# burchim/AVEC

Hardware: AMD Instinct MI355X
Metric: AV utterances/sec fwd+bwd (audio T=400, video 100x88x88) (higher is better)
Workload: dtype bf16

## Files before the change

### avec_amd/csrc/frontend.hip

```cpp
#include "vec.h"
#include "avec_hip.h"

__global__ __launch_bounds__(256) void mel_frames_kernel(const float* __restrict__ audio, const float* __restrict__ window, float* __restrict__ frames,
                                                         int B, long long L, int F, int n_fft, int win, int hop) {
  const long long total = (long long)B * F * win;
  const int off = (n_fft - win) / 2 - n_fft / 2;
  for (long long i = (long long)blockIdx.x * 256 + threadIdx.x; i < total; i += (long long)gridDim.x * 256) {
    const int n = (int)(i % win); const long long r = i / win; const int f = (int)(r % F); const long long b = r / F;
    long long s = (long long)f * hop + n + off;
    if (s < 0) s = -s; else if (s >= L) s = 2 * (L - 1) - s;
    frames[i] = audio[b * L + s] * window[n];
  }
}
__global__ __launch_bounds__(128) void mel_power_log_kernel(const float* __restrict__ spec, const float* __restrict__ fb, float* __restrict__ out,
                                                            int F, int nb, int n_mels) {
  extern __shared__ float pw[];
  const long long m = blockIdx.x; const int f = (int)(m % F); const long long b = m / F;
  for (int k = threadIdx.x; k < nb; k += 128) { const float re = spec[m * 2 * nb + k], im = spec[m * 2 * nb + nb + k]; pw[k] = re * re + im * im; }
  __syncthreads();
  for (int j = threadIdx.x; j < n_mels; j += 128) {
    float s = 0.f;
    for (int k = 0; k < nb; ++k) s += pw[k] * fb[k * n_mels + j];
    out[(b * n_mels + j) * F + f] = logf(s + 1e-9f);
  }
// ... 12 lines not shown

__global__ __launch_bounds__(256) void specaug_kernel(float* __restrict__ mel, const long long* __restrict__ lens, int B, int n_mels, int F, int mF, int Fp, int mT, float pS,
                                                      const unsigned long long* rng, unsigned stream) {
  const unsigned long long seed = rng[0] + 0x9e3779b97f4a7c15ull * rng[1];
  const long long total = (long long)B * n_mels * F;
  for (long long i = (long long)blockIdx.x * 256 + threadIdx.x; i < total; i += (long long)gridDim.x * 256) {
    const int f = (int)(i % F); const long long r = i / F; const int m = (int)(r % n_mels); const int b = (int)(r / n_mels);
    bool masked = false;
    for (int q = 0; q < mF && !masked; ++q) {
      const float val = rng_uniform(seed, stream, 2 * q) * Fp; const float mn = rng_uniform(seed, stream, 2 * q + 1) * (n_mels - val);
      const int s0 = (int)mn, s1 = (int)mn + (int)val; masked = (m >= s0 && m < s1);
    }
    const int len = lens ? (int)lens[b] : F; const int Tp = (int)(pS * len);
    if (f < len) for (int q = 0; q < mT && !masked; ++q) {
      const unsigned long long id = 1000ull + (unsigned long long)b * 64 + 2 * q;
      const float val = rng_uniform(seed, stream, id) * Tp; const float mn = rng_uniform(seed, stream, id + 1) * (len - val);
      const int s0 = (int)mn, s1 = (int)mn + (int)val; masked = (f >= s0 && f < s1);
    }
    if (masked) mel[i] = 0.f;
  }
}
extern "C" int avec_specaugment(float* mel, const long long* lens, int B, int n_mels, int F, int mF, int Fparam, int mT, float pS,
                                const unsigned long long* rng, unsigned rng_stream, hipStream_t st) {
  AVEC_CHECK_ARG(mel && rng && B > 0 && n_mels > 0 && F > 0, "specaugment: bad arguments");
  long long total = (long long)B * n_mels * F; long long nb = (total + 255) / 256; if (nb > 4096) nb = 4096;
  hipLaunchKernelGGL(specaug_kernel, dim3((unsigned)nb), dim3(256), 0, st, mel, lens, B, n_mels, F, mF, Fparam, mT, pS, rng, rng_stream);
  AVEC_LAUNCH_CHECK(); return 0;
}

__global__ void debug_rng_uniform_kernel(const unsigned long long* rng, unsigned stream, const long long* ids, int n, float* out) {
  const unsigned long long seed = rng[0] + 0x9e3779b97f4a7c15ull * rng[1];
  const int i = blockIdx.x * 256 + threadIdx.x;
  if (i < n) out[i] = rng_uniform(seed, stream, (unsigned long long)ids[i]);
}
extern "C" int avec_debug_rng_uniform(const unsigned long long* rng, unsigned rng_stream, const long long* ids, int n, float* out, hipStream_t st) {
  AVEC_CHECK_ARG(rng && ids && out && n > 0, "debug_rng_uniform: bad arguments");
  hipLaunchKernelGGL(debug_rng_uniform_kernel, dim3((n + 255) / 256), dim3(256), 0, st, rng, rng_stream, ids, n, out);
  AVEC_LAUNCH_CHECK(); return 0;
}

struct StemA { int B, NM, F, C, Fo, To; };

__device__ __forceinline__ void block_channel_add2(float* dst, int C, int c, bool live, float a, float b) {
  __shared__ float red[2][16]; __shared__ int cbase;
  if (threadIdx.x == 0) cbase = c;
  if (threadIdx.x < 32) red[threadIdx.x >> 4][threadIdx.x & 15] = 0.f;
  __syncthreads();
  const int k = c - cbase;
  if (live && k >= 0 && k < 16) { atomicAdd(&red[0][k], a); atomicAdd(&red[1][k], b); }
  else if (live) { atomicAdd(dst + c, a); atomicAdd(dst + C + c, b); }
  __syncthreads();
  if (threadIdx.x < 16 && cbase + (int)threadIdx.x < C && (red[0][threadIdx.x] != 0.f || red[1][threadIdx.x] != 0.f)) {
    atomicAdd(dst + cbase + threadIdx.x, red[0][threadIdx.x]); atomicAdd(dst + C + cbase + threadIdx.x, red[1][threadIdx.x]);
  }
}

template <typename T>
__global__ __launch_bounds__(256) void audio_stem_conv_kernel(const float* __restrict__ mel, const float* __restrict__ w, const float* __restrict__ bias,
                                                              T* __restrict__ y, float* stats, StemA s) {
  int j = blockIdx.x * 256 + threadIdx.x; const int J = s.C * s.Fo;
  const bool live = j < J; if (!live) j = J - 1;
  const int c = j / s.Fo, fo = j % s.Fo;
  float wk[9]; for (int q = 0; q < 9; ++q) wk[q] = w[c * 9 + q];
  const float bb = bias ? bias[c] : 0.f;
  float sum = 0.f, sq = 0.f;
  const long long M = (long long)s.B * s.To;
  for (long long row = blockIdx.y; row < M; row += gridDim.y) {
    const int to = (int)(row % s.To); const long long b = row / s.To;
    float acc = bb;
    for (int kh = 0; kh < 3; ++kh) { const int fi = 2 * fo + kh - 1; if (fi < 0 || fi >= s.NM) continue;
      for (int kw = 0; kw < 3; ++kw) { const int ti = 2 * to + kw - 1; if (ti < 0 || ti >= s.F) continue;
        acc += wk[kh * 3 + kw] * mel[(b * s.NM + fi) * s.F + ti]; } }
    if (live) { stf(y + row * J + j, acc); sum += acc; sq += acc * acc; }
  }
  if (stats) block_channel_add2(stats, s.C, c, live, sum, sq);
}
template <typename T>
__global__ __launch_bounds__(256) void audio_stem_act_kernel(const T* __restrict__ y, const float* __restrict__ ss, T* __restrict__ a, long long M, int J, int Fo, int C) {
  const long long total = M * J;
  for (long long i = (long long)blockIdx.x * 256 + threadIdx.x; i < total; i += (long long)gridDim.x * 256) {
    const int c = (int)((unsigned)(i % (long long)J)) / Fo; stf(a + i, swishf_(ldf(y + i) * ss[c] + ss[C + c]));
  }
}
template <typename T>
__global__ __launch_bounds__(256) void audio_stem_act8_kernel(const T* __restrict__ y, const float* __restrict__ ss, T* __restrict__ a, unsigned n8, unsigned J8, int Fo, int C) {
  for (unsigned i = blockIdx.x * 256 + threadIdx.x; i < n8; i += gridDim.x * 256) {
    const int c = (int)((i % J8) * 8) / Fo; const float sc = ss[c], sh = ss[C + c];
    Raw8<T> r; r.load(y + (long long)i * 8); float v[8]; r.get(v);
#pragma unroll
    for (int e = 0; e < 8; ++e) v[e] = swishf_(v[e] * sc + sh);
    st8<T>(a + (long long)i * 8, v);
  }
}
template <typename T>
__global__ __launch_bounds__(256) void audio_stem_bwd_reduce_kernel(const T* __restrict__ da, const T* __restrict__ y, const float* __restrict__ ss, float* dstats, StemA s) {
  int j = blockIdx.x * 256 + threadIdx.x; const int J = s.C * s.Fo;
  const bool live = j < J; if (!live) j = J - 1;
  const int c = j / s.Fo; const float sc = ss[c], sh = ss[s.C + c], mu = ss[2 * s.C + c], rs = ss[3 * s.C + c];
  float s1 = 0.f, s2 = 0.f; const long long M = (long long)s.B * s.To;
  if (live) for (long long row = blockIdx.y; row < M; row += gridDim.y) {
    const float yy = ldf(y + row * J + j); const float dr = ldf(da + row * J + j) * dswishf_(yy * sc + sh);
    s1 += dr; s2 += dr * (yy - mu) * rs;
  }
  block_channel_add2(dstats, s.C, c, live, s1, s2);
}
template <typename T>
__global__ __launch_bounds__(256) void audio_stem_bwd_params_kernel(const T* __restrict__ da, const T* __restrict__ y, const float* __restrict__ mel, const float* __restrict__ ss,
                                                                    const float* __restrict__ gamma, const float* __restrict__ dstats, const float* count_ptr, float count,
                                                                    float* dw, float* dbias, float* dgamma, float* dbeta, StemA s) {
  int j = blockIdx.x * 256 + threadIdx.x; const int J = s.C * s.Fo;
  const bool live = j < J; if (!live) j = J - 1;
  const int c = j / s.Fo, fo = j % s.Fo; const float inv_n = 1.f / (count_ptr ? *count_ptr : count);
  const float sc = ss[c], sh = ss[s.C + c], mu = ss[2 * s.C + c], rs = ss[3 * s.C + c], g = gamma[c];
  const float m1 = dstats[c] * inv_n, m2 = dstats[s.C + c] * inv_n;
  if (live && blockIdx.y == 0 && fo == 0 && dgamma) { atomicAdd(dgamma + c, dstats[s.C + c]); atomicAdd(dbeta + c, dstats[c]); }
  float aw[9]; for (int q = 0; q < 9; ++q) aw[q] = 0.f; float ab = 0.f;
  const long long M = (long long)s.B * s.To;
  if (live) for (long long row = blockIdx.y; row < M; row += gridDim.y) {
    const int to = (int)(row % s.To); const long long b = row / s.To;
    const float yy = ldf(y + row * J + j); const float dr = ldf(da + row * J + j) * dswishf_(yy * sc + sh);
    const float dy = g * rs * (dr - m1 - (yy - mu) * rs * m2);
    ab += dy;
    for (int kh = 0; kh < 3; ++kh) { const int fi = 2 * fo + kh - 1; if (fi < 0 || fi >= s.NM) continue;
      for (int kw = 0; kw < 3; ++kw) { const int ti = 2 * to + kw - 1; if (ti < 0 || ti >= s.F) continue;
        aw[kh * 3 + kw] += dy * mel[(b * s.NM + fi) * s.F + ti]; } }
  }
  __shared__ float wred[16][10]; __shared__ int wbase;
  if (threadIdx.x == 0) wbase = c;
  if (threadIdx.x < 160) wred[threadIdx.x / 10][threadIdx.x % 10] = 0.f;
  __syncthreads();
  const int kq = c - wbase;
  if (live && kq >= 0 && kq < 16) { for (int q = 0; q < 9; ++q) atomicAdd(&wred[kq][q], aw[q]); atomicAdd(&wred[kq][9], ab); }
  else if (live) { for (int q = 0; q < 9; ++q) atomicAdd(dw + c * 9 + q, aw[q]); if (dbias) atomicAdd(dbias + c, ab); }
  __syncthreads();
  if (threadIdx.x < 160) {
    const int cc = wbase + threadIdx.x / 10, q = threadIdx.x % 10; const float v = wred[threadIdx.x / 10][q];
    if (cc < s.C && v != 0.f) { if (q < 9) atomicAdd(dw + cc * 9 + q, v); else if (dbias) atomicAdd(dbias + cc, v); }
  }
}
#ifndef AVEC_AS_ROWS
#define AVEC_AS_ROWS 16
#endif
static constexpr int AS_ROWS = AVEC_AS_ROWS;
__device__ __forceinline__ void stage_mel_patch(float* patch, const float* mel, long long b, int to, const StemA& s) {
  for (int idx = threadIdx.x; idx < (s.NM + 2) * 3; idx += 256) {
    const int fi = idx / 3 - 1, kw = idx - (fi + 1) * 3; const int ti = 2 * to + kw - 1;
    patch[idx] = (fi >= 0 && fi < s.NM && ti >= 0 && ti < s.F) ? mel[(b * s.NM + fi) * s.F + ti] : 0.f;
  }
}
__device__ __forceinline__ void as_commit(const float* lsum, int n, float* const* dst, int ndst, int W, const ColWs& ws) {
  if (ws.partial) { float* mine = ws_slot(ws, 0, blockIdx.x, gridDim.x, n); for (int i = threadIdx.x; i < n; i += 256) mine[i] = lsum[i]; }
  else for (int i = threadIdx.x; i < n; i += 256) { const int q = i / W; if (dst[q] && lsum[i] != 0.f) atomicAdd(dst[q] + (i - q * W), lsum[i]); }
}
template <typename T>
__global__ __launch_bounds__(256) void audio_stem_conv8_kernel(const float* __restrict__ mel, const float* __restrict__ w, const float* __restrict__ bias,
                                                               T* __restrict__ y, float* stats, StemA s, ColWs ws) {
  extern __shared__ float asm_[];
  float* patch = asm_; float* lw = patch + (s.NM + 2) * 3; float* lsum = lw + s.C * 10;
  const int J = s.C * s.Fo, F8 = s.Fo >> 3, chunks = s.C * F8; const long long M = (long long)s.B * s.To;
  for (int i = threadIdx.x; i < s.C * 10; i += 256) { const int c = i / 10, q = i - c * 10; lw[i] = q < 9 ? w[c * 9 + q] : (bias ? bias[c] : 0.f); }
  for (int i = threadIdx.x; i < 2 * s.C; i += 256) lsum[i] = 0.f;
  for (int rr = 0; rr < AS_ROWS; ++rr) {
    const long long row = (long long)blockIdx.x * AS_ROWS + rr; if (row >= M) break;
    const int to = (int)(row % s.To); const long long b = row / s.To;
    __syncthreads();
    stage_mel_patch(patch, mel, b, to, s);
    __syncthreads();
    for (int ch = threadIdx.x; ch < chunks; ch += 256) {
      const int c = ch / F8, fo0 = (ch - c * F8) * 8; const float* wk = lw + c * 10;
      float acc[8], s1 = 0.f, s2 = 0.f;
#pragma unroll
      for (int e = 0; e < 8; ++e) {
        const float* pp = patch + (2 * (fo0 + e)) * 3; float a = wk[9];
// ... 41 lines not shown
  for (int rr = 0; rr < AS_ROWS; ++rr) {
    const long long row = (long long)blockIdx.x * AS_ROWS + rr; if (row >= M) break;
    const int to = (int)(row % s.To); const long long b = row / s.To;
    __syncthreads();
    stage_mel_patch(patch, mel, b, to, s);
    __syncthreads();
    for (int ch = threadIdx.x; ch < chunks; ch += 256) {
      const int c = ch / F8, fo0 = (ch - c * F8) * 8;
      const float sc = ss[c], sh = ss[s.C + c], mu = ss[2 * s.C + c], rs = ss[3 * s.C + c], g = gamma[c];
      const float m1 = dstats[c] * inv_n, m2 = dstats[s.C + c] * inv_n;
      float d[8], v[8], aw[9], ab = 0.f; ld8<T>(da + row * J + c * s.Fo + fo0, d); ld8<T>(y + row * J + c * s.Fo + fo0, v);
#pragma unroll
      for (int q = 0; q < 9; ++q) aw[q] = 0.f;
#pragma unroll
      for (int e = 0; e < 8; ++e) {
        const float dr = d[e] * dswishf_(v[e] * sc + sh); const float dy = g * rs * (dr - m1 - (v[e] - mu) * rs * m2);
        ab += dy; const float* pp = patch + (2 * (fo0 + e)) * 3;
#pragma unroll
        for (int q = 0; q < 9; ++q) aw[q] += dy * pp[q];
      }
#pragma unroll
      for (int q = 0; q < 9; ++q) atomicAdd(lsum + q * s.C + c, aw[q]);
      atomicAdd(lsum + 9 * s.C + c, ab);
    }
  }
  __syncthreads();
  if (ws.partial) { float* mine = ws_slot(ws, 0, blockIdx.x, gridDim.x, 10 * s.C); for (int i = threadIdx.x; i < 10 * s.C; i += 256) mine[i] = lsum[i]; }
  else for (int i = threadIdx.x; i < 10 * s.C; i += 256) { const int q = i / s.C, c = i - q * s.C; if (q < 9) atomicAdd(dw + c * 9 + q, lsum[i]); else if (dbias) atomicAdd(dbias + c, lsum[i]); }
}
constexpr int AS_NIT = 4;
__device__ __forceinline__ void as_patch51(const float* patch, int fo0, float p[52]) {
  const float4* q = (const float4*)(patch + 6 * fo0);
#pragma unroll
  for (int k = 0; k < 13; ++k) { const float4 t = q[k]; p[4 * k] = t.x; p[4 * k + 1] = t.y; p[4 * k + 2] = t.z; p[4 * k + 3] = t.w; }
}
template <typename T>
__global__ __launch_bounds__(256) void audio_stem_conv8x_kernel(const float* __restrict__ mel, const float* __restrict__ w, const float* __restrict__ bias,
                                                                T* __restrict__ y, float* stats, StemA s, ColWs ws) {
  extern __shared__ __attribute__((aligned(16))) float asm_[];
  float* patch = asm_; float* lsum = patch + (((s.NM + 2) * 3 + 4 + 3) & ~3);
  const int J = s.C * s.Fo, F8 = s.Fo >> 3, chunks = s.C * F8; const long long M = (long long)s.B * s.To;
  int cc[AS_NIT], fo[AS_NIT]; float wk[AS_NIT][10], s1[AS_NIT], s2[AS_NIT];
#pragma unroll
  for (int it = 0; it < AS_NIT; ++it) {
    const int ch = threadIdx.x + 256 * it; const bool ok = ch < chunks; cc[it] = ok ? ch / F8 : -1; fo[it] = ok ? (ch - cc[it] * F8) * 8 : 0; s1[it] = s2[it] = 0.f;
#pragma unroll
    for (int q = 0; q < 10; ++q) wk[it][q] = ok ? (q < 9 ? w[cc[it] * 9 + q] : (bias ? bias[cc[it]] : 0.f)) : 0.f;
  }
  for (int i = threadIdx.x; i < 2 * s.C; i += 256) lsum[i] = 0.f;
  for (int rr = 0; rr < AS_ROWS; ++rr) {
    const long long row = (long long)blockIdx.x * AS_ROWS + rr; if (row >= M) break;
    const int to = (int)(row % s.To); const long long b = row / s.To;
    __syncthreads();
    stage_mel_patch(patch, mel, b, to, s);
    __syncthreads();
#pragma unroll
    for (int it = 0; it < AS_NIT; ++it) {
      if (cc[it] < 0) continue;
      float p[52], acc[8]; as_patch51(patch, fo[it], p);
#pragma unroll
      for (int e = 0; e < 8; ++e) {
        float a = wk[it][9];
#pragma unroll
        for (int q = 0; q < 9; ++q) a += wk[it][q] * p[6 * e + q];
        acc[e] = a; s1[it] += a; s2[it] += a * a;
      }
      st8<T>(y + row * J + cc[it] * s.Fo + fo[it], acc);
    }
  }
  if (!stats) return;
#pragma unroll
  for (int it = 0; it < AS_NIT; ++it) if (cc[it] >= 0) { atomicAdd(lsum + cc[it], s1[it]); atomicAdd(lsum + s.C + cc[it], s2[it]); }
  __syncthreads();
  float* const dst[2] = {stats, stats + s.C}; as_commit(lsum, 2 * s.C, dst, 2, s.C, ws);
}
template <typename T>
__global__ __launch_bounds__(256) void audio_stem_bwd_reduce8x_kernel(const T* __restrict__ da, const T* __restrict__ y, const float* __restrict__ ss, float* dstats, StemA s, ColWs ws) {
  extern __shared__ __attribute__((aligned(16))) float asm_[];
  float* lsum = asm_;
  const int J = s.C * s.Fo, F8 = s.Fo >> 3, chunks = s.C * F8; const long long M = (long long)s.B * s.To;
  int cc[AS_NIT], off[AS_NIT]; float sc[AS_NIT], sh[AS_NIT], mu[AS_NIT], rs[AS_NIT], s1[AS_NIT], s2[AS_NIT];
#pragma unroll
  for (int it = 0; it < AS_NIT; ++it) {
    const int ch = threadIdx.x + 256 * it; const bool ok = ch < chunks; const int c = ok ? ch / F8 : 0; cc[it] = ok ? c : -1; off[it] = c * s.Fo + (ch - c * F8) * 8;
    sc[it] = ss[c]; sh[it] = ss[s.C + c]; mu[it] = ss[2 * s.C + c]; rs[it] = ss[3 * s.C + c]; s1[it] = s2[it] = 0.f;
  }
  for (int i = threadIdx.x; i < 2 * s.C; i += 256) lsum[i] = 0.f;
  for (int rr = 0; rr < AS_ROWS; ++rr) {
    const long long row = (long long)blockIdx.x * AS_ROWS + rr; if (row >= M) break;
    Raw8<T> rd[AS_NIT], rv[AS_NIT];
#pragma unroll
    for (int it = 0; it < AS_NIT; ++it) if (cc[it] >= 0) { rd[it].load(da + row * J + off[it]); rv[it].load(y + row * J + off[it]); }
#pragma unroll
    for (int it = 0; it < AS_NIT; ++it) {
      if (cc[it] < 0) continue;
      float d[8], v[8]; rd[it].get(d); rv[it].get(v);
#pragma unroll
      for (int e = 0; e < 8; ++e) { const float dr = d[e] * dswishf_(v[e] * sc[it] + sh[it]); s1[it] += dr; s2[it] += dr * (v[e] - mu[it]) * rs[it]; }
    }
  }
  __syncthreads();
#pragma unroll
  for (int it = 0; it < AS_NIT; ++it) if (cc[it] >= 0) { atomicAdd(lsum + cc[it], s1[it]); atomicAdd(lsum + s.C + cc[it], s2[it]); }
  __syncthreads();
  float* const dst[2] = {dstats, dstats + s.C}; as_commit(lsum, 2 * s.C, dst, 2, s.C, ws);
}
template <typename T>
__global__ __launch_bounds__(256) void audio_stem_bwd_params8x_kernel(const T* __restrict__ da, const T* __restrict__ y, const float* __restrict__ mel, const float* __restrict__ ss,
                                                                      const float* __restrict__ gamma, const float* __restrict__ dstats, const float* count_ptr, float count,
                                                                      float* dw, float* dbias, float* dgamma, float* dbeta, StemA s, ColWs ws) {
  extern __shared__ __attribute__((aligned(16))) float asm_[];
  float* patch = asm_; float* lsum = patch + (((s.NM + 2) * 3 + 4 + 3) & ~3);
  const int J = s.C * s.Fo, F8 = s.Fo >> 3, chunks = s.C * F8; const long long M = (long long)s.B * s.To;
  const float inv_n = 1.f / (count_ptr ? *count_ptr : count);
  if (blockIdx.x == 0 && dgamma) for (int c = threadIdx.x; c < s.C; c += 256) { atomicAdd(dgamma + c, dstats[s.C + c]); atomicAdd(dbeta + c, dstats[c]); }
  int cc[AS_NIT], fo[AS_NIT]; float sc[AS_NIT], sh[AS_NIT], mu[AS_NIT], A[AS_NIT], m1[AS_NIT], rm2[AS_NIT], aw[AS_NIT][10];
#pragma unroll
  for (int it = 0; it < AS_NIT; ++it) {
    const int ch = threadIdx.x + 256 * it; const bool ok = ch < chunks; const int c = ok ? ch / F8 : 0; cc[it] = ok ? c : -1; fo[it] = ok ? (ch - c * F8) * 8 : 0;
    const float rs = ss[3 * s.C + c];
    sc[it] = ss[c]; sh[it] = ss[s.C + c]; mu[it] = ss[2 * s.C + c]; A[it] = gamma[c] * rs; m1[it] = dstats[c] * inv_n; rm2[it] = rs * dstats[s.C + c] * inv_n;
#pragma unroll
    for (int q = 0; q < 10; ++q) aw[it][q] = 0.f;
  }
  for (int i = threadIdx.x; i < 10 * s.C; i += 256) lsum[i] = 0.f;
  for (int rr = 0; rr < AS_ROWS; ++rr) {
    const long long row = (long long)blockIdx.x * AS_ROWS + rr; if (row >= M) break;
    const int to = (int)(row % s.To); const long long b = row / s.To;
    Raw8<T> rd[AS_NIT], rv[AS_NIT];
#pragma unroll
    for (int it = 0; it < AS_NIT; ++it) if (cc[it] >= 0) { const long long o = row * J + cc[it] * s.Fo + fo[it]; rd[it].load(da + o); rv[it].load(y + o); }
    __syncthreads();
    stage_mel_patch(patch, mel, b, to, s);
    __syncthreads();
#pragma unroll
    for (int it = 0; it < AS_NIT; ++it) {
      if (cc[it] < 0) continue;
      float d[8], v[8], p[52]; rd[it].get(d); rv[it].get(v); as_patch51(patch, fo[it], p);
#pragma unroll
      for (int e = 0; e < 8; ++e) {
        const float dr = d[e] * dswishf_(v[e] * sc[it] + sh[it]); const float dy = A[it] * (dr - m1[it] - (v[e] - mu[it]) * rm2[it]);
        aw[it][9] += dy;
#pragma unroll
        for (int q = 0; q < 9; ++q) aw[it][q] += dy * p[6 * e + q];
      }
    }
  }
  __syncthreads();
#pragma unroll
  for (int it = 0; it < AS_NIT; ++it) if (cc[it] >= 0) {
#pragma unroll
    for (int q = 0; q < 10; ++q) atomicAdd(lsum + q * s.C + cc[it], aw[it][q]);
  }
  __syncthreads();
  if (ws.partial) { float* mine = ws_slot(ws, 0, blockIdx.x, gridDim.x, 10 * s.C); for (int i = threadIdx.x; i < 10 * s.C; i += 256) mine[i] = lsum[i]; }
  else for (int i = threadIdx.x; i < 10 * s.C; i += 256) { const int q = i / s.C, c = i - q * s.C; if (q < 9) atomicAdd(dw + c * 9 + q, lsum[i]); else if (dbias) atomicAdd(dbias + c, lsum[i]); }
}
static bool as8x_ok(const StemA& s) { return s.C * (s.Fo >> 3) <= AS_NIT * 256; }
static bool as8_ok(const StemA& s) { return s.Fo % 8 == 0 && ((size_t)(s.NM + 2) * 3 + (size_t)s.C * 12) * 4 <= 60 * 1024; }
static unsigned as8_blocks(const StemA& s) { return (unsigned)(((long long)s.B * s.To + AS_ROWS - 1) / AS_ROWS); }
static StemA stemA(int B, int NM, int F, int C) { StemA s; s.B = B; s.NM = NM; s.F = F; s.C = C; s.Fo = (NM - 1) / 2 + 1; s.To = (F - 1) / 2 + 1; return s; }
static dim3 stem_grid(const StemA& s) { long long M = (long long)s.B * s.To; unsigned gx = (s.C * s.Fo + 255) / 256; long long gy = 2048 / gx; if (gy > M) gy = M; if (gy < 1) gy = 1; return dim3(gx, (unsigned)gy); }

extern "C" int avec_audio_stem_conv_fwd(int dtype, const float* mel, const float* w, const float* bias, void* y, float* stats, int B, int n_mels, int F, int C, hipStream_t st) {
  AVEC_CHECK_ARG(mel && w && y && B > 0 && n_mels > 0 && F > 0 && C > 0, "audio_stem_conv_fwd: bad arguments");
  StemA s = stemA(B, n_mels, F, C);
  if (as8_ok(s)) {
    const unsigned nb = as8_blocks(s); const ColPlan plan = ColPlan::flat<2>(nb, C, st, stats != nullptr);
    const size_t lds = ((size_t)(n_mels + 2) * 3 + (size_t)C * 12) * 4;
    if (as8x_ok(s)) { const size_t l2 = ((size_t)(((n_mels + 2) * 3 + 4 + 3) & ~3) + (size_t)C * 2) * 4;
      DISPATCH_T(dtype, hipLaunchKernelGGL(audio_stem_conv8x_kernel<T>, dim3(nb), dim3(256), l2, st, mel, w, bias, (T*)y, stats, s, plan.ws)); }
    else
    DISPATCH_T(dtype, hipLaunchKernelGGL(audio_stem_conv8_kernel<T>, dim3(nb), dim3(256), lds, st, mel, w, bias, (T*)y, stats, s, plan.ws));
    AVEC_LAUNCH_CHECK();
    return plan.finish({stats, stats + C}, C, st);
  }
  DISPATCH_T(dtype, hipLaunchKernelGGL(audio_stem_conv_kernel<T>, stem_grid(s), dim3(256), 0, st, mel, w, bias, (T*)y, stats, s));
  AVEC_LAUNCH_CHECK(); return 0;
}
extern "C" int avec_audio_stem_act_fwd(int dtype, const void* y, const float* ss, void* a, int B, int n_mels, int F, int C, hipStream_t st) {
  AVEC_CHECK_ARG(y && ss && a, "audio_stem_act_fwd: null pointer");
  StemA s = stemA(B, n_mels, F, C); long long M = (long long)B * s.To; long long nb = (M * C * s.Fo + 255) / 256; if (nb > 4096) nb = 4096;
  if (s.Fo % 8 == 0 && M * C * s.Fo / 8 < (1ll << 31)) {
    const long long n8 = M * C * s.Fo / 8; long long nb8 = (n8 + 255) / 256; if (nb8 > 8192) nb8 = 8192;
    DISPATCH_T(dtype, hipLaunchKernelGGL(audio_stem_act8_kernel<T>, dim3((unsigned)nb8), dim3(256), 0, st, (const T*)y, ss, (T*)a, (unsigned)n8, (unsigned)(C * s.Fo / 8), s.Fo, C));
    AVEC_LAUNCH_CHECK(); return 0;
  }
  DISPATCH_T(dtype, hipLaunchKernelGGL(audio_stem_act_kernel<T>, dim3((unsigned)nb), dim3(256), 0, st, (const T*)y, ss, (T*)a, M, C * s.Fo, s.Fo, C));
  AVEC_LAUNCH_CHECK(); return 0;
}
extern "C" int avec_audio_stem_bwd(int dtype, const void* da, const void* y, const float* mel, const float* ss, const float* gamma, float* dstats,
                                   const float* count_ptr, float count, int phase, float* dw, float* dbias, float* dgamma, float* dbeta,
                                   int B, int n_mels, int F, int C, hipStream_t st) {
  AVEC_CHECK_ARG(da && y && mel && ss && gamma && dstats && (phase == 0 || (dw != nullptr)), "audio_stem_bwd: bad arguments");
  StemA s = stemA(B, n_mels, F, C);
  if (as8_ok(s)) {
    const unsigned nb = as8_blocks(s);
    if (phase == 0) {
      const ColPlan plan = ColPlan::flat<2>(nb, C, st);
      if (as8x_ok(s)) DISPATCH_T(dtype, hipLaunchKernelGGL(audio_stem_bwd_reduce8x_kernel<T>, dim3(nb), dim3(256), (size_t)2 * C * 4, st, (const T*)da, (const T*)y, ss, dstats, s, plan.ws));
      else
      DISPATCH_T(dtype, hipLaunchKernelGGL(audio_stem_bwd_reduce8_kernel<T>, dim3(nb), dim3(256), (size_t)2 * C * 4, st, (const T*)da, (const T*)y, ss, dstats, s, plan.ws));
      AVEC_LAUNCH_CHECK();
      return plan.finish({dstats, dstats + C}, C, st);
    } else {
      const ColPlan plan = ColPlan::flat<10>(nb, C, st);
      const size_t lds = ((size_t)(n_mels + 2) * 3 + (size_t)C * 10) * 4;
      if (as8x_ok(s)) { const size_t l2 = ((size_t)(((n_mels + 2) * 3 + 4 + 3) & ~3) + (size_t)C * 10) * 4;
        DISPATCH_T(dtype, hipLaunchKernelGGL(audio_stem_bwd_params8x_kernel<T>, dim3(nb), dim3(256), l2, st, (const T*)da, (const T*)y, mel, ss, gamma, dstats, count_ptr, count,
                                             dw, dbias, dgamma, dbeta, s, plan.ws)); }
      else
      DISPATCH_T(dtype, hipLaunchKernelGGL(audio_stem_bwd_params8_kernel<T>, dim3(nb), dim3(256), lds, st, (const T*)da, (const T*)y, mel, ss, gamma, dstats, count_ptr, count,
                                           dw, dbias, dgamma, dbeta, s, plan.ws));
      AVEC_LAUNCH_CHECK();
      float* dst[10]; for (int q = 0; q < 9; ++q) dst[q] = dw + q; dst[9] = nullptr;
      if (int r = plan.finish(dst, C, st, 9)) return r;
      for (int q = 0; q < 9; ++q) dst[q] = nullptr; dst[9] = dbias;
      return dbias ? plan.finish(dst, C, st) : 0;
    }
  }
  if (phase == 0) { DISPATCH_T(dtype, hipLaunchKernelGGL(audio_stem_bwd_reduce_kernel<T>, stem_grid(s), dim3(256), 0, st, (const T*)da, (const T*)y, ss, dstats, s)); }
  else { DISPATCH_T(dtype, hipLaunchKernelGGL(audio_stem_bwd_params_kernel<T>, stem_grid(s), dim3(256), 0, st, (const T*)da, (const T*)y, mel, ss, gamma, dstats, count_ptr, count, dw, dbias, dgamma, dbeta, s)); }
  AVEC_LAUNCH_CHECK(); return 0;
}

template <typename T>
__global__ __launch_bounds__(256) void stem_pool_fwd_kernel(const T* __restrict__ y, const float* __restrict__ ss, T* __restrict__ out, unsigned char* __restrict__ idx,
                                                            T* __restrict__ ymax, long long Fr, int H, int W, int C, int OH, int OW) {
  const long long n4 = Fr * OH * OW * (C / 4);
  for (long long i = (long long)blockIdx.x * 256 + threadIdx.x; i < n4; i += (long long)gridDim.x * 256) {
    const unsigned iu = (unsigned)i, C4 = (unsigned)C >> 2;
    const int c = (int)(iu % C4) * 4; unsigned r = iu / C4; const int ow = (int)(r % (unsigned)OW); r /= (unsigned)OW; const int oh = (int)(r % (unsigned)OH); const long long fr = r / (unsigned)OH;
    float sc[4], sh[4]; ld4<float>(ss + c, sc); ld4<float>(ss + C + c, sh);
    float best[4] = {0.f, 0.f, 0.f, 0.f}, braw[4] = {0.f, 0.f, 0.f, 0.f}; unsigned bi[4] = {255u, 255u, 255u, 255u};
    float v[9][4]; bool ok[9];
#pragma unroll
    for (int q = 0; q < 9; ++q) {
      const int kh = q / 3, kw = q - kh * 3; const int h = 2 * oh + kh - 1, w = 2 * ow + kw - 1;
      ok[q] = h >= 0 && h < H && w >= 0 && w < W;
      ld4<T>(y + ((fr * H + (ok[q] ? h : 0)) * W + (ok[q] ? w : 0)) * C + c, v[q]);
    }
#pragma unroll
    for (int q = 0; q < 9; ++q)
      for (int e = 0; e < 4; ++e) { const float a = v[q][e] * sc[e] + sh[e]; if (ok[q] && a > best[e]) { best[e] = a; bi[e] = q; braw[e] = v[q][e]; } }
    st4<T>(out + i * 4, best);
    if (ymax) st4<T>(ymax + i * 4, braw);
    *(uint32_t*)(idx + i * 4) = bi[0] | (bi[1] << 8) | (bi[2] << 16) | (bi[3] << 24);
  }
}
template <typename T>
__device__ __forceinline__ void stem_dr(const T* dp, const unsigned char* idx, long long fr, int h, int w, int c, int C, int OH, int OW, float dr[4]) {
  dr[0] = dr[1] = dr[2] = dr[3] = 0.f;
  for (int kh = 0; kh < 3; ++kh) { const int t = h + 1 - kh; if (t < 0 || (t & 1)) continue; const int oh = t >> 1; if (oh >= OH) continue;
    for (int kw = 0; kw < 3; ++kw) { const int u = w + 1 - kw; if (u < 0 || (u & 1)) continue; const int ow = u >> 1; if (ow >= OW) continue;
      const long long o = ((fr * OH + oh) * OW + ow) * C + c;
      const uint32_t sel = *(const uint32_t*)(idx + o); float g[4]; ld4<T>(dp + o, g);
      for (int e = 0; e < 4; ++e) if (((sel >> (8 * e)) & 255u) == (unsigned)(kh * 3 + kw)) dr[e] += g[e]; } }
}
template <typename T>
__global__ __launch_bounds__(256) void stem_pool_bwd_reduce_kernel(const T* __restrict__ dp, const unsigned char* __restrict__ idx, const T* __restrict__ y, const float* __restrict__ ss,
                                                                   float* dstats, long long Fr, int H, int W, int C, int OH, int OW, ColWs ws) {
  const int tx = threadIdx.x & 31, ty = threadIdx.x >> 5; const int col = (blockIdx.x * 32 + tx) * 4;
  float part[2][4] = {{0.f, 0.f, 0.f, 0.f}, {0.f, 0.f, 0.f, 0.f}};
  const long long M = Fr * H * W;
  if (col < C) {
    float mu[4], rs[4]; ld4<float>(ss + 2 * C + col, mu); ld4<float>(ss + 3 * C + col, rs);
    for (long long row = (long long)blockIdx.y * 8 + ty; row < M; row += (long long)gridDim.y * 8) {
// ... 197 lines not shown
```

### avec_amd/csrc/norm.hip

```cpp
#include "common.h"
#include "avec_hip.h"

#include "vec.h"
#include <type_traits>

__global__ __launch_bounds__(256) void col_finalize_kernel(ColFin f) {
  __shared__ float red[16][17];
  const int cw = threadIdx.x & 15, sl = threadIdx.x >> 4;
  const int ncols = f.NV * f.W;
  const int o = blockIdx.x * 16 + cw;
  const unsigned cb = blockIdx.y;
  const int s0 = blockIdx.z * 128;
  float s = 0.f;
  if (o < ncols) {
    const float* p = f.partial + ((size_t)cb * f.nslots) * ncols + o;
#pragma unroll
    for (int k = 0; k < 8; ++k) {
      const int si = s0 + sl + 16 * k; const int sc = si < f.nslots ? si : f.nslots - 1;
      const float v = p[(size_t)sc * ncols];
      s += si < f.nslots ? v : 0.f;
    }
  }
  red[sl][cw] = s;
  __syncthreads();
// ... 190 lines not shown
  norm(g2, b2, eps2, mean2, rstd2);
#pragma unroll
  for (int i = 0; i < 2; ++i) { const int c = lane * 4 + i * 256; if (c < D) st4<TO>(h2 + row * D + c, v[i]); }
}
extern "C" int avec_layernorm_fwd2(int dtype, const float* x, const float* gamma1, const float* beta1, float eps1, float* y1, float* mean1, float* rstd1,
                                   const float* gamma2, const float* beta2, float eps2, void* h2, float* mean2, float* rstd2, long long M, int D, hipStream_t st) {
  AVEC_CHECK_ARG(x && gamma1 && beta1 && y1 && mean1 && rstd1 && gamma2 && beta2 && h2 && mean2 && rstd2, "layernorm_fwd2: null pointer");
  AVEC_CHECK_ARG(M > 0 && D > 0 && D % 4 == 0 && D <= 512, "layernorm_fwd2: D=%d must be a multiple of 4 in [4, 512]", D);
  dim3 grid((unsigned)((M + 3) / 4));
  if (dtype == AVEC_F32) hipLaunchKernelGGL(ln_fwd2_kernel<float>, grid, dim3(256), 0, st, x, gamma1, beta1, eps1, y1, mean1, rstd1, gamma2, beta2, eps2, (float*)h2, mean2, rstd2, M, D);
  else hipLaunchKernelGGL(ln_fwd2_kernel<bf16>, grid, dim3(256), 0, st, x, gamma1, beta1, eps1, y1, mean1, rstd1, gamma2, beta2, eps2, (bf16*)h2, mean2, rstd2, M, D);
  AVEC_LAUNCH_CHECK(); return 0;
}
template <typename TG>
__global__ __launch_bounds__(256) void ln_bwd_rows2_kernel(const TG* __restrict__ dy2, const float* __restrict__ x2, const float* __restrict__ mean2, const float* __restrict__ rstd2,
                                                           const float* __restrict__ g2, const float* __restrict__ dres2, float* __restrict__ dx2,
                                                           const float* __restrict__ x1, const float* __restrict__ mean1, const float* __restrict__ rstd1,
                                                           const float* __restrict__ g1, float* __restrict__ dx1, long long M, int D, LnPrep pr) {
  const int lane = threadIdx.x & 63; const long long row = (long long)blockIdx.x * 4 + (threadIdx.x >> 6);
  if (row >= M) return;
  float d[2][4], v[2][4], o[2][4], gg[2][4], w1[2][4], gg1[2][4];
  const float mu2 = mean2[row], rs2 = rstd2[row], mu1 = mean1[row], rs1 = rstd1[row];
  DropKey dk; dk.k0 = 0u; dk.thr = 0u; dk.scale = 1.f;
  if (pr.out) dk = drop_key(pr.rng, pr.stream, pr.p);
#pragma unroll
  for (int i = 0; i < 2; ++i) {
    const int c = lane * 4 + i * 256;
    if (c < D) {
      ld4<TG>(dy2 + row * D + c, d[i]); ld4<float>(x2 + row * D + c, v[i]); ld4<float>(g2 + c, gg[i]); ld4<float>(x1 + row * D + c, w1[i]); ld4<float>(g1 + c, gg1[i]);
      if (dres2) ld4<float>(dres2 + row * D + c, o[i]); else { o[i][0] = o[i][1] = o[i][2] = o[i][3] = 0.f; }
    } else {
#pragma unroll
      for (int e = 0; e < 4; ++e) { d[i][e] = 0.f; v[i][e] = mu2; o[i][e] = 0.f; gg[i][e] = 0.f; w1[i][e] = mu1; gg1[i][e] = 0.f; }
    }
  }
  float s1 = 0.f, s2 = 0.f;
#pragma unroll
  for (int i = 0; i < 2; ++i)
#pragma unroll
    for (int e = 0; e < 4; ++e) { const float xh = (v[i][e] - mu2) * rs2, t = d[i][e] * gg[i][e]; v[i][e] = xh; s1 += t; s2 += t * xh; }
  s1 = wave_sum(s1) / D; s2 = wave_sum(s2) / D;
#pragma unroll
  for (int i = 0; i < 2; ++i) {
    const int c = lane * 4 + i * 256;
#pragma unroll
    for (int e = 0; e < 4; ++e) o[i][e] += rs2 * (d[i][e] * gg[i][e] - s1 - v[i][e] * s2);
    if (c < D) st4<float>(dx2 + row * D + c, o[i]); else { o[i][0] = o[i][1] = o[i][2] = o[i][3] = 0.f; }
  }
  float t1 = 0.f, t2 = 0.f;
#pragma unroll
  for (int i = 0; i < 2; ++i)
#pragma unroll
    for (int e = 0; e < 4; ++e) { const float xh = (w1[i][e] - mu1) * rs1, t = o[i][e] * gg1[i][e]; w1[i][e] = xh; t1 += t; t2 += t * xh; }
  t1 = wave_sum(t1) / D; t2 = wave_sum(t2) / D;
#pragma unroll
  for (int i = 0; i < 2; ++i) {
    const int c = lane * 4 + i * 256; if (c >= D) break;
    float r[4];
#pragma unroll
    for (int e = 0; e < 4; ++e) r[e] = rs1 * (o[i][e] * gg1[i][e] - t1 - w1[i][e] * t2);
    st4<float>(dx1 + row * D + c, r);
    if (pr.out) {
      float q[4], ds[4]; drop4(dk, (unsigned long long)row * D + c, ds);
#pragma unroll
      for (int e = 0; e < 4; ++e) q[e] = r[e] * (pr.alpha * ds[e]);
      if (pr.f32) st4<float>((float*)pr.out + row * D + c, q); else st4<bf16>((bf16*)pr.out + row * D + c, q);
    }
  }
}
extern "C" int avec_layernorm_bwd2(int dtype, const void* dy2, const float* x2, const float* mean2, const float* rstd2, const float* gamma2, const float* dres2, float* dx2,
                                   const float* x1, const float* mean1, const float* rstd1, const float* gamma1, float* dx1,
                                   void* prep, float prep_alpha, float prep_drop_p, const unsigned long long* rng, unsigned rng_stream, long long M, int D, hipStream_t st) {
  AVEC_CHECK_ARG(dy2 && x2 && mean2 && rstd2 && gamma2 && dx2 && x1 && mean1 && rstd1 && gamma1 && dx1, "layernorm_bwd2: null pointer");
  AVEC_CHECK_ARG(M > 0 && D > 0 && D % 4 == 0 && D <= 512 && (!prep || prep_drop_p <= 0.f || rng), "layernorm_bwd2: D=%d must be a multiple of 4 in [4, 512]; dropout needs rng", D);
  LnPrep pr; pr.out = prep; pr.alpha = prep_alpha; pr.p = prep ? prep_drop_p : 0.f; pr.rng = rng; pr.stream = rng_stream; pr.f32 = dtype == AVEC_F32;
  dim3 grid((unsigned)((M + 3) / 4));
  if (dtype == AVEC_F32) hipLaunchKernelGGL(ln_bwd_rows2_kernel<float>, grid, dim3(256), 0, st, (const float*)dy2, x2, mean2, rstd2, gamma2, dres2, dx2, x1, mean1, rstd1, gamma1, dx1, M, D, pr);
  else hipLaunchKernelGGL(ln_bwd_rows2_kernel<bf16>, grid, dim3(256), 0, st, (const bf16*)dy2, x2, mean2, rstd2, gamma2, dres2, dx2, x1, mean1, rstd1, gamma1, dx1, M, D, pr);
  AVEC_LAUNCH_CHECK(); return 0;
}

struct LnItem { const void* dy; const float* x; const float* mean; const float* rstd; float* dg; float* db; int M, D, dy_f32, first; };
struct LnGroup { LnItem it[AVEC_LN_GROUP_MAX]; int n; };
static constexpr int LNG_ROWS = 128;
__global__ __launch_bounds__(256) void ln_param_grads_grouped_kernel(LnGroup grp) {
  __shared__ float red[2][256][4];
  const int w = blockIdx.x;
  int lo = 0, hi = grp.n - 1;
  while (lo < hi) { const int mid = (lo + hi + 1) >> 1; if (grp.it[mid].first <= w) lo = mid; else hi = mid - 1; }
  const LnItem& t = grp.it[lo];
  const int D = t.D, L = D >> 2, R = 256 / L;
  const int r = threadIdx.x / L, l = threadIdx.x - r * L;
  const int m0 = (w - t.first) * LNG_ROWS; int m1 = m0 + LNG_ROWS; if (m1 > t.M) m1 = t.M;
  float pg[4] = {0.f, 0.f, 0.f, 0.f}, pb[4] = {0.f, 0.f, 0.f, 0.f};
  if (r < R) {
    constexpr int U = 8;
    for (int m = m0 + r; m < m1; m += R * U) {
      float d[U][4], v[U][4], mu[U], rs[U];
#pragma unroll
      for (int u = 0; u < U; ++u) {
        const int mm = m + u * R; const bool ok = mm < m1; const long long mi = ok ? mm : m;
        if (t.dy_f32) ld4<float>((const float*)t.dy + mi * D + l * 4, d[u]); else ld4<bf16>((const bf16*)t.dy + mi * D + l * 4, d[u]);
        ld4<float>(t.x + mi * D + l * 4, v[u]); mu[u] = t.mean[mi]; rs[u] = ok ? t.rstd[mi] : 0.f;
        if (!ok) d[u][0] = d[u][1] = d[u][2] = d[u][3] = 0.f;
      }
#pragma unroll
      for (int u = 0; u < U; ++u)
#pragma unroll
        for (int e = 0; e < 4; ++e) { pg[e] += d[u][e] * (v[u][e] - mu[u]) * rs[u]; pb[e] += d[u][e]; }
    }
  }
#pragma unroll
  for (int e = 0; e < 4; ++e) { red[0][threadIdx.x][e] = pg[e]; red[1][threadIdx.x][e] = pb[e]; }
  __syncthreads();
  for (int o = threadIdx.x; o < 2 * D; o += 256) {
    const int which = o >= D, c = o - which * D; float s = 0.f;
    for (int rr = 0; rr < R; ++rr) s += red[which][rr * L + (c >> 2)][c & 3];
    atomicAdd((which ? t.db : t.dg) + c, s);
  }
}
extern "C" int avec_layernorm_param_grads_grouped(int dtype, const avec_ln_item_t* items, int n, hipStream_t st) {
  AVEC_CHECK_ARG(items && n > 0 && n <= AVEC_LN_GROUP_MAX, "layernorm_param_grads_grouped: need 1..%d items (got %d)", AVEC_LN_GROUP_MAX, n);
  LnGroup grp; grp.n = n; int first = 0;
  for (int k = 0; k < n; ++k) {
    const avec_ln_item_t& s = items[k];
    AVEC_CHECK_ARG(s.dy && s.x && s.mean && s.rstd && s.dgamma && s.dbeta && s.M > 0 && s.M < (1ll << 31) && s.D >= 4 && s.D % 4 == 0 && s.D <= 1024,
                   "layernorm_param_grads_grouped: item %d: null pointer or D=%d not a multiple of 4 in [4, 1024]", k, s.D);
    LnItem& t = grp.it[k];
    t.dy = s.dy; t.x = s.x; t.mean = s.mean; t.rstd = s.rstd; t.dg = s.dgamma; t.db = s.dbeta; t.M = (int)s.M; t.D = s.D;
    t.dy_f32 = (s.dy_f32 || dtype == AVEC_F32) ? 1 : 0; t.first = first;
    first += (int)((s.M + LNG_ROWS - 1) / LNG_ROWS);
  }
  hipLaunchKernelGGL(ln_param_grads_grouped_kernel, dim3((unsigned)first), dim3(256), 0, st, grp);
  AVEC_LAUNCH_CHECK(); return 0;
}

static int layernorm_bwd_impl(int dtype, const void* dy, int dy_f32, const float* x, const float* mean, const float* rstd, const float* gamma,
                              float* dx, const float* dres, float* dgamma, float* dbeta, long long M, int D, const LnPrep& pr, hipStream_t st) {
  AVEC_CHECK_ARG(dy && x && mean && rstd && gamma && dx && (!dgamma == !dbeta), "layernorm_bwd: null pointer");
  AVEC_CHECK_ARG(M > 0 && D > 0 && D % 4 == 0 && D <= 1536, "layernorm_bwd: D=%d must be a multiple of 4 and <= 1536", D);
  AVEC_CHECK_ARG(!pr.out || (!dgamma && (pr.p <= 0.f || pr.rng)), "layernorm_bwd_prep: the second output comes with the dx-only kernel (dgamma == NULL); dropout needs rng");
  if (!dgamma) {
    const dim3 grid((unsigned)((M + 3) / 4)); const bool f32in = dy_f32 || dtype == AVEC_F32;
#define AVEC_LN_ROWS(TG, NG) hipLaunchKernelGGL((ln_bwd_rows_kernel<TG, NG>), grid, dim3(256), 0, st, (const TG*)dy, x, mean, rstd, gamma, dx, dres, M, D, pr)
    if (D <= 512) { if (f32in) AVEC_LN_ROWS(float, 2); else AVEC_LN_ROWS(bf16, 2); }
    else { if (f32in) AVEC_LN_ROWS(float, 6); else AVEC_LN_ROWS(bf16, 6); }
#undef AVEC_LN_ROWS
    AVEC_LAUNCH_CHECK(); return 0;
  }
  long long nb = (M + 15) / 16; if (nb > 256) nb = 256; if (nb < 1) nb = 1;
  const ColPlan plan = ColPlan::flat<2>((unsigned)nb, D, st).cap_without_ws(128);
  const size_t lds = (size_t)2 * D * sizeof(float);
#define AVEC_LN_BWD(TG, NG) hipLaunchKernelGGL((ln_bwd_kernel<TG, NG>), dim3(plan.nslots), dim3(256), lds, st, (const TG*)dy, x, mean, rstd, gamma, dx, dres, dgamma, dbeta, M, D, plan.ws)
  const bool f32in = dy_f32 || dtype == AVEC_F32;
  if (D <= 512) { if (f32in) AVEC_LN_BWD(float, 2); else AVEC_LN_BWD(bf16, 2); }
  else { if (f32in) AVEC_LN_BWD(float, 6); else AVEC_LN_BWD(bf16, 6); }
#undef AVEC_LN_BWD
  AVEC_LAUNCH_CHECK();
  return plan.finish({dgamma, dbeta}, D, st);
}
extern "C" int avec_layernorm_bwd(int dtype, const void* dy, int dy_f32, const float* x, const float* mean, const float* rstd, const float* gamma,
                                  float* dx, const float* dres, float* dgamma, float* dbeta, long long M, int D, hipStream_t st) {
  LnPrep pr; pr.out = nullptr; pr.alpha = 1.f; pr.p = 0.f; pr.rng = nullptr; pr.stream = 0; pr.f32 = 0;
  return layernorm_bwd_impl(dtype, dy, dy_f32, x, mean, rstd, gamma, dx, dres, dgamma, dbeta, M, D, pr, st);
}
extern "C" int avec_layernorm_bwd_prep(int dtype, const void* dy, int dy_f32, const float* x, const float* mean, const float* rstd, const float* gamma,
                                       float* dx, const float* dres, void* prep, float prep_alpha, float prep_drop_p, const unsigned long long* rng, unsigned rng_stream,
                                       long long M, int D, hipStream_t st) {
  AVEC_CHECK_ARG(prep, "layernorm_bwd_prep: null prep buffer");
  LnPrep pr; pr.out = prep; pr.alpha = prep_alpha; pr.p = prep_drop_p; pr.rng = rng; pr.stream = rng_stream; pr.f32 = dtype == AVEC_F32;
  return layernorm_bwd_impl(dtype, dy, dy_f32, x, mean, rstd, gamma, dx, dres, nullptr, nullptr, M, D, pr, st);
}

template <typename T>
__global__ __launch_bounds__(256) void grad_prep_kernel(const float* __restrict__ dout, long long ldd, T* __restrict__ dacc, float alpha, float p,
                                                        const unsigned long long* rng, unsigned stream, float* dbias, long long M, int N, ColWs ws) {
  const int tx = threadIdx.x & 31, ty = threadIdx.x >> 5;
  const int col = (blockIdx.x * 32 + tx) * 4;
  float part[1][4] = {{0.f, 0.f, 0.f, 0.f}};
  const DropKey dk = drop_key(rng, stream, p);
  if (col < N) {
    for (long long row = (long long)blockIdx.y * 8 + ty; row < M; row += (long long)gridDim.y * 8) {
      float v[4]; ld4<float>(dout + row * ldd + col, v);
      float ds[4]; drop4(dk, (unsigned long long)row * N + col, ds);
      for (int e = 0; e < 4; ++e) { v[e] *= alpha * ds[e]; part[0][e] += v[e]; }
      st4<T>(dacc + row * N + col, v);
    }
  }
  float* const dst[1] = {dbias};
  if (dbias) colreduce_atomic<1>(part, dst, col, N, ws);
}

template <typename T>
__global__ __launch_bounds__(256) void grad_prep_flat_kernel(const float* __restrict__ dout, long long ldd, T* __restrict__ dacc, float alpha, float p,
                                                             const unsigned long long* rng, unsigned stream, long long M, int N) {
  const int N4 = N >> 2; const long long n4 = M * N4;
  const DropKey dk = drop_key(rng, stream, p);
  for (long long i = (long long)blockIdx.x * 256 + threadIdx.x; i < n4; i += (long long)gridDim.x * 256) {
    const long long row = n4 < (1ll << 31) ? (long long)((unsigned)i / (unsigned)N4) : i / N4; const int col = (int)(i - row * N4) * 4;
    float v[4]; ld4<float>(dout + row * ldd + col, v);
    float ds[4]; drop4(dk, (unsigned long long)row * N + col, ds);
    for (int e = 0; e < 4; ++e) v[e] *= alpha * ds[e];
    st4<T>(dacc + row * N + col, v);
// ... 788 lines not shown
```

Before: 1944.

## Batch and prefetch loads in audio stem and layernorm param-grad kernels

The audio stem activation kernel now processes four chunks per thread, issuing all loads before computing, with nontemporal loads for bf16 and a grid sized to cover everything with no grid-stride loop. The stem backward reduce kernel double-buffers row loads so the next row's fetch overlaps the current row's math. The layernorm grouped param-grad kernel hoists the dtype branch into a templated helper and uses nontemporal vector loads. The aim is more memory-level parallelism and less cache pollution in bandwidth-bound kernels, at the cost of higher register pressure and a larger grid.

```diff
diff --git a/avec_amd/csrc/frontend.hip b/avec_amd/csrc/frontend.hip
--- a/avec_amd/csrc/frontend.hip
+++ b/avec_amd/csrc/frontend.hip
@@ -118,13 +118,27 @@
     const int c = (int)((unsigned)(i % (long long)J)) / Fo; stf(a + i, swishf_(ldf(y + i) * ss[c] + ss[C + c]));
   }
 }
+constexpr int AS_ACT_P = 4;
+template <typename T> __device__ __forceinline__ void as_ld_nt(Raw8<T>& r, const T* p) { r.load(p); }
+template <> __device__ __forceinline__ void as_ld_nt<bf16>(Raw8<bf16>& r, const bf16* p) {
+  typedef unsigned v4u __attribute__((ext_vector_type(4))); const v4u t = __builtin_nontemporal_load((const v4u*)p); r.t = make_uint4(t.x, t.y, t.z, t.w);
+}
 template <typename T>
 __global__ __launch_bounds__(256) void audio_stem_act8_kernel(const T* __restrict__ y, const float* __restrict__ ss, T* __restrict__ a, unsigned n8, unsigned J8, int Fo, int C) {
-  for (unsigned i = blockIdx.x * 256 + threadIdx.x; i < n8; i += gridDim.x * 256) {
-    const int c = (int)((i % J8) * 8) / Fo; const float sc = ss[c], sh = ss[C + c];
-    Raw8<T> r; r.load(y + (long long)i * 8); float v[8]; r.get(v);
-#pragma unroll
-    for (int e = 0; e < 8; ++e) v[e] = swishf_(v[e] * sc + sh);
+  const unsigned base = blockIdx.x * (256u * AS_ACT_P) + threadIdx.x;
+  Raw8<T> r[AS_ACT_P]; float sc[AS_ACT_P], sh[AS_ACT_P];
+#pragma unroll
+  for (int p = 0; p < AS_ACT_P; ++p) {
+    const unsigned i = base + p * 256; const unsigned j = i < n8 ? i : n8 - 1;
+    as_ld_nt<T>(r[p], y + (long long)j * 8);
+    const int c = (int)((j % J8) * 8) / Fo; sc[p] = ss[c]; sh[p] = ss[C + c];
+  }
+#pragma unroll
+  for (int p = 0; p < AS_ACT_P; ++p) {
+    const unsigned i = base + p * 256; if (i >= n8) break;
+    float v[8]; r[p].get(v);
+#pragma unroll
+    for (int e = 0; e < 8; ++e) v[e] = swishf_(v[e] * sc[p] + sh[p]);
     st8<T>(a + (long long)i * 8, v);
   }
 }
@@ -332,22 +346,33 @@
   int cc[AS_NIT], off[AS_NIT]; float sc[AS_NIT], sh[AS_NIT], mu[AS_NIT], rs[AS_NIT], s1[AS_NIT], s2[AS_NIT];
 #pragma unroll
   for (int it = 0; it < AS_NIT; ++it) {
-    const int ch = threadIdx.x + 256 * it; const bool ok = ch < chunks; const int c = ok ? ch / F8 : 0; cc[it] = ok ? c : -1; off[it] = c * s.Fo + (ch - c * F8) * 8;
+    const int ch = threadIdx.x + 256 * it; const bool ok = ch < chunks; const int chv = ok ? ch : chunks - 1; const int c = chv / F8; cc[it] = ok ? c : -1;
+    off[it] = c * s.Fo + (chv - c * F8) * 8;
     sc[it] = ss[c]; sh[it] = ss[s.C + c]; mu[it] = ss[2 * s.C + c]; rs[it] = ss[3 * s.C + c]; s1[it] = s2[it] = 0.f;
   }
   for (int i = threadIdx.x; i < 2 * s.C; i += 256) lsum[i] = 0.f;
-  for (int rr = 0; rr < AS_ROWS; ++rr) {
-    const long long row = (long long)blockIdx.x * AS_ROWS + rr; if (row >= M) break;
-    Raw8<T> rd[AS_NIT], rv[AS_NIT];
-#pragma unroll
-    for (int it = 0; it < AS_NIT; ++it) if (cc[it] >= 0) { rd[it].load(da + row * J + off[it]); rv[it].load(y + row * J + off[it]); }
+  struct Row { Raw8<T> d[AS_NIT], v[AS_NIT]; };
+  const long long row0 = (long long)blockIdx.x * AS_ROWS; const int nrows = (int)(M - row0 < AS_ROWS ? M - row0 : AS_ROWS);
+  auto fetch = [&](int rr, Row& r) {
+    const long long o = (row0 + (rr < nrows ? rr : nrows - 1)) * J;
+#pragma unroll
+    for (int it = 0; it < AS_NIT; ++it) { r.d[it].load(da + o + off[it]); r.v[it].load(y + o + off[it]); }
+  };
+  auto use = [&](const Row& r) {
 #pragma unroll
     for (int it = 0; it < AS_NIT; ++it) {
       if (cc[it] < 0) continue;
-      float d[8], v[8]; rd[it].get(d); rv[it].get(v);
+      float d[8], v[8]; r.d[it].get(d); r.v[it].get(v);
 #pragma unroll
       for (int e = 0; e < 8; ++e) { const float dr = d[e] * dswishf_(v[e] * sc[it] + sh[it]); s1[it] += dr; s2[it] += dr * (v[e] - mu[it]) * rs[it]; }
     }
+  };
+  Row ra, rb;
+  if (nrows > 0) fetch(0, ra);
+  for (int rr = 0; rr < nrows; rr += 2) {
+    fetch(rr + 1, rb); use(ra);
+    if (rr + 1 >= nrows) break;
+    fetch(rr + 2, ra); use(rb);
   }
   __syncthreads();
 #pragma unroll
@@ -432,7 +457,7 @@
   AVEC_CHECK_ARG(y && ss && a, "audio_stem_act_fwd: null pointer");
   StemA s = stemA(B, n_mels, F, C); long long M = (long long)B * s.To; long long nb = (M * C * s.Fo + 255) / 256; if (nb > 4096) nb = 4096;
   if (s.Fo % 8 == 0 && M * C * s.Fo / 8 < (1ll << 31)) {
-    const long long n8 = M * C * s.Fo / 8; long long nb8 = (n8 + 255) / 256; if (nb8 > 8192) nb8 = 8192;
+    const long long n8 = M * C * s.Fo / 8; const long long nb8 = (n8 + 256 * AS_ACT_P - 1) / (256 * AS_ACT_P);
     DISPATCH_T(dtype, hipLaunchKernelGGL(audio_stem_act8_kernel<T>, dim3((unsigned)nb8), dim3(256), 0, st, (const T*)y, ss, (T*)a, (unsigned)n8, (unsigned)(C * s.Fo / 8), s.Fo, C));
     AVEC_LAUNCH_CHECK(); return 0;
   }
diff --git a/avec_amd/csrc/norm.hip b/avec_amd/csrc/norm.hip
--- a/avec_amd/csrc/norm.hip
+++ b/avec_amd/csrc/norm.hip
@@ -296,7 +296,33 @@
 
 struct LnItem { const void* dy; const float* x; const float* mean; const float* rstd; float* dg; float* db; int M, D, dy_f32, first; };
 struct LnGroup { LnItem it[AVEC_LN_GROUP_MAX]; int n; };
+static constexpr int LNG_U = 8;
 static constexpr int LNG_ROWS = 128;
+__device__ __forceinline__ void lng_ld(const float* p, float v[4]) {
+  typedef float v4f __attribute__((ext_vector_type(4))); const v4f t = __builtin_nontemporal_load((const v4f*)p); v[0] = t.x; v[1] = t.y; v[2] = t.z; v[3] = t.w;
+}
+__device__ __forceinline__ void lng_ld(const bf16* p, float v[4]) {
+  typedef unsigned v2u __attribute__((ext_vector_type(2))); const v2u t = __builtin_nontemporal_load((const v2u*)p);
+  v[0] = __uint_as_float(t.x << 16); v[1] = __uint_as_float(t.x & 0xffff0000u); v[2] = __uint_as_float(t.y << 16); v[3] = __uint_as_float(t.y & 0xffff0000u);
+}
+template <typename TG>
+__device__ __forceinline__ void lng_sum_rows(const LnItem& t, int m0, int m1, int r, int R, int l, float (&pg)[4], float (&pb)[4]) {
+  const int D = t.D; const TG* dy = (const TG*)t.dy;
+  for (int m = m0 + r; m < m1; m += R * LNG_U) {
+    float d[LNG_U][4], v[LNG_U][4], mu[LNG_U], rs[LNG_U];
+#pragma unroll
+    for (int u = 0; u < LNG_U; ++u) {
+      const int mm = m + u * R; const long long mi = mm < m1 ? mm : m;
+      lng_ld(dy + mi * D + l * 4, d[u]); lng_ld(t.x + mi * D + l * 4, v[u]); mu[u] = t.mean[mi]; rs[u] = t.rstd[mi];
+    }
+#pragma unroll
+    for (int u = 0; u < LNG_U; ++u) {
+      const bool ok = m + u * R < m1; const float rsu = ok ? rs[u] : 0.f;
+#pragma unroll
+      for (int e = 0; e < 4; ++e) { const float de = ok ? d[u][e] : 0.f; pg[e] += de * (v[u][e] - mu[u]) * rsu; pb[e] += de; }
+    }
+  }
+}
 __global__ __launch_bounds__(256) void ln_param_grads_grouped_kernel(LnGroup grp) {
   __shared__ float red[2][256][4];
   const int w = blockIdx.x;
@@ -307,23 +333,7 @@
   const int r = threadIdx.x / L, l = threadIdx.x - r * L;
   const int m0 = (w - t.first) * LNG_ROWS; int m1 = m0 + LNG_ROWS; if (m1 > t.M) m1 = t.M;
   float pg[4] = {0.f, 0.f, 0.f, 0.f}, pb[4] = {0.f, 0.f, 0.f, 0.f};
-  if (r < R) {
-    constexpr int U = 8;
-    for (int m = m0 + r; m < m1; m += R * U) {
-      float d[U][4], v[U][4], mu[U], rs[U];
-#pragma unroll
-      for (int u = 0; u < U; ++u) {
-        const int mm = m + u * R; const bool ok = mm < m1; const long long mi = ok ? mm : m;
-        if (t.dy_f32) ld4<float>((const float*)t.dy + mi * D + l * 4, d[u]); else ld4<bf16>((const bf16*)t.dy + mi * D + l * 4, d[u]);
-        ld4<float>(t.x + mi * D + l * 4, v[u]); mu[u] = t.mean[mi]; rs[u] = ok ? t.rstd[mi] : 0.f;
-        if (!ok) d[u][0] = d[u][1] = d[u][2] = d[u][3] = 0.f;
-      }
-#pragma unroll
-      for (int u = 0; u < U; ++u)
-#pragma unroll
-        for (int e = 0; e < 4; ++e) { pg[e] += d[u][e] * (v[u][e] - mu[u]) * rs[u]; pb[e] += d[u][e]; }
-    }
-  }
+  if (r < R) { if (t.dy_f32) lng_sum_rows<float>(t, m0, m1, r, R, l, pg, pb); else lng_sum_rows<bf16>(t, m0, m1, r, R, l, pg, pb); }
 #pragma unroll
   for (int e = 0; e < 4; ++e) { red[0][threadIdx.x][e] = pg[e]; red[1][threadIdx.x][e] = pb[e]; }
   __syncthreads();
@@ -333,6 +343,7 @@
     atomicAdd((which ? t.db : t.dg) + c, s);
   }
 }
+extern "C" int avec_layernorm_param_grads_rows(int D) { return D >= 4 && D % 4 == 0 && D <= 1024 ? LNG_ROWS : 0; }
 extern "C" int avec_layernorm_param_grads_grouped(int dtype, const avec_ln_item_t* items, int n, hipStream_t st) {
   AVEC_CHECK_ARG(items && n > 0 && n <= AVEC_LN_GROUP_MAX, "layernorm_param_grads_grouped: need 1..%d items (got %d)", AVEC_LN_GROUP_MAX, n);
   LnGroup grp; grp.n = n; int first = 0;
```

Measured after the change: 1942. Within noise of the previous version (-0.1%).
